# yhw-yhw/TalkSHOW

Hardware: NVIDIA H100
Metric: smplx_motion_frames_per_sec (higher is better)
Workload: dtype f32

## Files before the change

### talkshow_b200/csrc/api.cu

```cuda
#include "convstack.h"
#include "pixelcnn.h"

using namespace ts;

static std::string g_create_err;

float* ts_engine::upload(const std::vector<float>& h) {
  if (host_only) return nullptr;
  void* d = dmalloc(h.size() * sizeof(float));
  TS_CUDA(cudaMemcpy(d, h.data(), h.size() * sizeof(float), cudaMemcpyHostToDevice));
  return (float*)d;
}
unsigned short* ts_engine::upload(const std::vector<unsigned short>& h) {
  if (host_only) return nullptr;
  void* d = dmalloc(h.size() * sizeof(unsigned short));
  TS_CUDA(cudaMemcpy(d, h.data(), h.size() * sizeof(unsigned short), cudaMemcpyHostToDevice));
  return (unsigned short*)d;
}
void* ts_engine::dmalloc(size_t bytes) {
  if (host_only) return nullptr;
  void* d = nullptr;
  TS_CUDA(cudaMalloc(&d, bytes ? bytes : 16));
  (alloc_sink ? *alloc_sink : owned).push_back(d);
  return d;
// ... 60 lines not shown

extern "C" int ts_set_pixelcnn_ctas(ts_engine* e, int n) {
  if (!e || n < 0) return TS_ERR_INVALID;
  e->pixel_ctas = n;
  return TS_OK;
}

extern "C" int ts_set_vq_parallel(ts_engine* e, int max_batch) {
  if (!e || max_batch < 0) return TS_ERR_INVALID;
  e->vq_parallel_batch = max_batch;
  return TS_OK;
}

extern "C" int ts_set_pixelcnn_fusion(ts_engine* e, int on) {
  if (!e) return TS_ERR_INVALID;
  if (on < 0 || on > 2) return TS_ERR_INVALID;
  e->pixel_fusion = on;
  return TS_OK;
}

__constant__ float c_lower_pose[33] = {0.0f, 0.0f, 0.0f, 0.0f, 0.0f, 0.0f, 3.0747f, -0.0158f, -0.0152f,
    -1.1826512813568115f, 0.23866955935955048f, 0.15146760642528534f, -1.2604516744613647f, -0.3160211145877838f,
    -0.1603458970785141f, 1.1654603481292725f, 0.0f, 0.0f, 1.2521806955337524f, 0.041598282754421234f,
    -0.06312154978513718f, 0.0f, 0.0f, 0.0f, 0.0f, 0.0f, 0.0f, 0.0f, 0.0f, 0.0f, 0.0f, 0.0f, 0.0f};

__device__ __forceinline__ void rot6d_to_aa(const float* __restrict__ p, float& ax, float& ay, float& az) {
  const float a1x = p[0], a1y = p[1], a1z = p[2], a2x = p[3], a2y = p[4], a2z = p[5];
  float n1 = fmaxf(sqrtf(a1x * a1x + a1y * a1y + a1z * a1z), 1e-12f);
  const float b1x = a1x / n1, b1y = a1y / n1, b1z = a1z / n1;
  const float d = b1x * a2x + b1y * a2y + b1z * a2z;
  float b2x = a2x - d * b1x, b2y = a2y - d * b1y, b2z = a2z - d * b1z;
// ... 215 lines not shown
```

### talkshow_b200/csrc/pixelcnn.cu

```cuda
#include "pixelcnn.h"
#include "convstack.h"

#include <algorithm>
#include <memory>
#include <cmath>

namespace ts {


struct Job {
  int epi, layer, col, nrows, K, ncol;
  bool pairs;
  int rofs = 0;
};

constexpr double PIX_ROWCOST = 0.0;

static int rows_cap(int K) { return std::min(PIX_MAXROWS, (PIX_WBUF / (K + 1)) & ~3); }

static void push_vert0(std::vector<std::vector<Job>>& st, int D, bool split) {
  if (split) {
    st.push_back({{EPI_VERT0, 0, 0, 2 * D, 6 * D, 1, true}});
    st.push_back({{EPI_VERT0, 0, 1, 2 * D, 6 * D, 1, true}});
  } else {
// ... 13 lines not shown
  }
  for (int c = 0; c < 2; ++c) {
    std::vector<Job> j = {{EPI_HRESF, 0, c, D, D, 1, false}};
    if (c == 0) j.push_back({EPI_V2H, L - 1, 0, 2 * D, 2 * D, 2, false});
    st.push_back(j);
    st.push_back({{EPI_HGATE, 1, c, 2 * D, c ? 2 * D : D, 1, true}});
    for (int l = 2; l < L; ++l)
      st.push_back({{EPI_HGATE2, l, c, 2 * D, c ? 3 * D : 2 * D, 1, true}, {EPI_HRES, l - 1, c, D, D, 1, false}});
    st.push_back({{EPI_OUT1F, 0, c, 512, 2 * D, 1, false}});
    for (int q = 0; q < out2_split; ++q) st.push_back({{EPI_OUT2, 0, c, PIX_NCODE / out2_split, 512, 1, false, q * (PIX_NCODE / out2_split)}});
    st.push_back({{EPI_SAMPLE, 0, c, 0, c == 0 ? 1 : 0, 1, false}});
  }
  return st;
}

static std::vector<std::vector<Job>> build_stages_fused2(int L, int D = PIX_D, int out2_split = 1, bool v0_split = false) {
  std::vector<std::vector<Job>> st;
  push_vert0(st, D, v0_split);
  st.push_back({{EPI_FUSEV, 0, 0, D, D, 2, false}, {EPI_V2H, 0, 0, 2 * D, 2 * D, 2, false}});
  for (int l = 1; l < L; ++l) {
    std::vector<Job> j = {{EPI_VERT, l, 0, 2 * D, 4 * D, 1, true}, {EPI_VERT, l, 1, 2 * D, 4 * D, 1, true}};
    if (l == 1) j.push_back({EPI_HGATE, 0, 0, 2 * D, 0, 1, true});
    st.push_back(j);
  }
  for (int c = 0; c < 2; ++c) {
    st.push_back({{EPI_HRESF, 0, c, D, D, 1, false}, {EPI_V2H1, 1, c, 2 * D, 2 * D, 1, false}});
    {
      std::vector<Job> j = {{EPI_HGATE, 1, c, 2 * D, c ? 2 * D : D, 1, true}};
      if (L > 2) j.push_back({EPI_V2H1, 2, c, 2 * D, 2 * D, 1, false});
      st.push_back(j);
// ... 22 lines not shown
  for (int c = 0; c < 2; ++c) {
    std::vector<Job> j = {{EPI_HGATE, 0, c, 2 * D, c ? D : 0, 1, true}};
    if (c == 0) j.push_back({EPI_V2H, L - 1, 0, 2 * D, 2 * D, 2, false});
    st.push_back(j);
    st.push_back({{EPI_HRES, 0, c, D, D, 1, false}});
    st.push_back({{EPI_FUSEH, 0, c, D, D, 1, false}});
    for (int l = 1; l < L; ++l) {
      st.push_back({{EPI_HGATE, l, c, 2 * D, c ? 2 * D : D, 1, true}});
      st.push_back({{EPI_HRES, l, c, D, D, 1, false}});
    }
    st.push_back({{EPI_OUT1, 0, c, 512, D, 1, false}});
    st.push_back({{EPI_OUT2, 0, c, PIX_NCODE, 512, 1, false}});
    st.push_back({{EPI_SAMPLE, 0, c, 0, 0, 1, false}});
  }
  return st;
}

static PixLayout make_layout(int L, int hvslots, int MB = PIX_MB) {
  PixLayout a;
  int o = 0;
  auto take = [&](int nseg) { int r = o; o += nseg * PIX_D * MB; return r; };
  a.E = take(4 * 2);
  a.XV1P = take(2);
  a.XV = take(L * 2 * 2);
  a.HV = take(hvslots * 2 * 2);
  a.V2H = take(L * 2 * 2);
  a.G = take(2);
  a.XHP = take(1);
  a.XH = take(2 * (L + 1));
  a.Y = take(2);
// ... 150 lines not shown
  if (e->pixel_ctas > 0) {
    if (e->pixel_ctas < PIX_MB || e->pixel_ctas > e->sm_count) {
      const int n = e->pixel_ctas, sms = e->sm_count;
      fail(TS_ERR_UNSUPPORTED, "pixelcnn plan: ts_set_pixelcnn_ctas(%d) outside [%d, %d] (one CTA per sample of a 64-sample tile; SM count)", n, PIX_MB, sms);
    }
    P->ncta = e->pixel_ctas & ~1;
  }
  if (const char* v = getenv("TS_PIX_CTAS")) {
    const int n = atoi(v);
    if (n >= PIX_MB && n <= e->sm_count) P->ncta = n;
  }
  P->cl = cl;
  P->nclasses = ncls;
  bool fused = level >= 1 && L >= 3;
  P->sched = fused ? level : 0;
  P->lay = make_layout(L, P->sched == 2 ? L : 2);
  if (P->ncta < PIX_MB) fail(TS_ERR_UNSUPPORTED, "pixelcnn plan needs >= %d SMs (have %d)", PIX_MB, P->ncta);
  P->fused = fused;
  const int out2_split = (PIX_NCODE + PIX_MAXROWS * P->ncta - 1) / (PIX_MAXROWS * P->ncta);
  if (out2_split > 1 && !fused) fail(TS_ERR_UNSUPPORTED, "pixelcnn plan: %d CTAs need the fused plan", P->ncta);
  const bool v0_split = fused && 2 * cdiv(2 * D, rows_cap(6 * D)) > P->ncta / cl;
  auto stages = P->sched == 2 ? build_stages_fused2(L, PIX_D, out2_split, v0_split)
                : fused       ? build_stages_fused(L, PIX_D, out2_split, v0_split)
                              : build_stages(L);
  P->nstages = (int)stages.size();
  if (P->nstages > 160) fail(TS_ERR_UNSUPPORTED, "pixelcnn plan: %d stages per row (> 160)", P->nstages);
  P->table.assign((size_t)P->nstages * P->ncta, PixTask{0, 0, 0, 0, 0, 0, 0, 0});
  WeightSrc ws(ck, L);
  if (fused) ws.build_fused();
  int64_t dense = 0;
  int t0_ofs = 0;
  if (fused) {
    const float* ew = ck.f32("embedding.weight", {PIX_NCODE, D});
    const Job j0{EPI_HGATE, 0, 1, 2 * D, D, 1, true};
    P->blob.resize((size_t)PIX_NCODE * 2 * D);
    std::vector<float> wrow((size_t)2 * D * D), brow(2 * D);
    for (int jr = 0; jr < 2 * D; ++jr) {
      brow[jr] = ws.bias(j0, jr);
      for (int k = 0; k < D; ++k) wrow[(size_t)jr * D + k] = ws.w(j0, jr, k);
    }
    for (int code = 0; code < PIX_NCODE; ++code)
      for (int jr = 0; jr < 2 * D; ++jr) {
        double a = 0.0;
        for (int k = 0; k < D; ++k) a += (double)wrow[(size_t)jr * D + k] * (double)ew[(size_t)code * D + k];
        P->blob[(size_t)code * 2 * D + jr] = (float)(a + (double)brow[jr]);
      }
  }
  const size_t table_floats = P->blob.size();
  for (int s = 0; s < P->nstages; ++s) {
    auto& jobs = stages[s];
    if (jobs[0].epi == EPI_SAMPLE) {
      for (int c = 0; c < P->ncta; ++c)
        P->table[(size_t)s * P->ncta + c] = PixTask{EPI_SAMPLE, 0, jobs[0].col, 0, 0, jobs[0].K ? t0_ofs : 0, jobs[0].K, 0};
      continue;
    }
    std::vector<double> cost;
    double tot = 0;
    const double alpha = getenv("TS_PIX_ROWCOST") ? atof(getenv("TS_PIX_ROWCOST")) : PIX_ROWCOST;
    for (auto& j : jobs) { double c = (double)j.nrows * (j.K ? std::max(j.K, 256) + alpha : 16) * j.ncol; cost.push_back(c); tot += c; }
    std::vector<int> nc(jobs.size()), lo(jobs.size());
    int used = 0;
    const int nunit = P->ncta / cl;
    const int rowcap = PIX_MAXROWS;
    for (size_t i = 0; i < jobs.size(); ++i) {
      const int cap = jobs[i].K ? rows_cap(jobs[i].K / cl) : 4 * PIX_MAXROWS;
      lo[i] = (jobs[i].nrows + cap - 1) / cap;
      nc[i] = std::max(lo[i], (int)std::floor(nunit * cost[i] / tot));
      used += nc[i];
    }
    for (size_t i = 0; used < nunit; i = (i + 1) % jobs.size()) { nc[i]++; used++; }
    while (used > nunit) {
      size_t big = 0; int slack = -1;
      for (size_t i = 0; i < jobs.size(); ++i) if (nc[i] - lo[i] > slack) { slack = nc[i] - lo[i]; big = i; }
      if (slack <= 0) fail(TS_ERR_UNSUPPORTED, "pixelcnn plan: %d SMs are too few for stage %d", P->ncta, s);
      nc[big]--; used--;
    }
    int cta = 0;
    for (size_t i = 0; i < jobs.size(); ++i) {
      const Job& j = jobs[i];
      const int unit = j.pairs ? 2 : 1, units = j.nrows / unit;
      const int base = units / nc[i], rem = units % nc[i];
      int u0 = 0;
      for (int q = 0; q < nc[i]; ++q) {
        int nu = base + (q < rem ? 1 : 0);
        for (int rank = 0; rank < cl; ++rank, ++cta) {
          PixTask t{0, 0, 0, 0, 0, 0, 0, 0};
          if (nu > 0) {
            t.epi = j.epi; t.layer = j.layer; t.col = j.col;
            t.row0 = j.rofs + u0 * unit; t.nrows = nu * unit; t.K = j.K; t.rpad = (t.nrows + 3) & ~3;
            if (t.K > 0 && t.nrows > rowcap) fail(TS_ERR_UNSUPPORTED, "pixelcnn plan: %d rows per unit (> %d) with %d SMs", t.nrows, rowcap, P->ncta);
            const int Ks = t.K / cl, k0 = rank * Ks;
            size_t sz = (size_t)(Ks + 1) * t.rpad;
            if (sz > (size_t)PIX_WBUF) fail(TS_ERR_UNSUPPORTED, "pixelcnn plan: task blob %zu floats > staging buffer", sz);
            t.wofs = (int)P->blob.size();
            P->blob.resize(P->blob.size() + sz, 0.f);
            float* dst = P->blob.data() + t.wofs;
            for (int r = 0; r < t.nrows; ++r) {
              for (int k = 0; k < Ks; ++k) dst[(size_t)k * t.rpad + r] = ws.w(j, t.row0 - j.rofs + r, k0 + k);
              dst[(size_t)Ks * t.rpad + r] = ws.bias(j, t.row0 - j.rofs + r);
            }
            dense += (int64_t)t.nrows * Ks;
          }
          P->table[(size_t)s * P->ncta + cta] = t;
        }
        u0 += nu;
      }
    }
  }
  P->staged_row_bytes = 4 * ((int64_t)(P->blob.size() - table_floats) + 3LL * D * D);
  (void)dense;
  P->has_v1 = true;

  if (!e->host_only) {
    P->d_table = (PixTask*)e->dmalloc(P->table.size() * sizeof(PixTask));
    TS_CUDA(cudaMemcpy(P->d_table, P->table.data(), P->table.size() * sizeof(PixTask), cudaMemcpyHostToDevice));
    P->d_blob = e->upload(P->blob);
    const float* ew = ck.f32("embedding.weight", {PIX_NCODE, D});
    P->d_emb = e->upload(std::vector<float>(ew, ew + (size_t)PIX_NCODE * D));
    std::vector<float> cls((size_t)L * ncls * 2 * D);
// ... 19 lines not shown
  const int64_t* pre;
  int64_t* idx_out;
  float* logits_out;
  unsigned* barrier;
  PixLayout lay;
  int B, T0, Ttot, log_r0, L, nstages, ncta, fused;
  unsigned long long* trace;
  int trace_row;
  float temperature;
  int top_k;
  float* logp_out;
  float top_p, min_p;
  int* kept_out;
  const int64_t* seeds;
  const int64_t* anchors;
};

__device__ __forceinline__ uint32_t smem_u32(const void* p) { return (uint32_t)__cvta_generic_to_shared(p); }
__device__ __forceinline__ void mbar_init(uint64_t* bar, int count) {
  asm volatile("mbarrier.init.shared::cta.b64 [%0], %1;" ::"r"(smem_u32(bar)), "r"(count));
}
__device__ __forceinline__ void mbar_expect_tx(uint64_t* bar, uint32_t bytes) {
  asm volatile("mbarrier.arrive.expect_tx.shared::cta.b64 _, [%0], %1;" ::"r"(smem_u32(bar)), "r"(bytes) : "memory");
}
__device__ __forceinline__ void mbar_wait(uint64_t* bar, uint32_t parity) {
  asm volatile(
      "{\n"
      ".reg .pred p;\n"
      "WAIT_LOOP:\n"
      "mbarrier.try_wait.parity.shared::cta.b64 p, [%0], %1;\n"
// ... 322 lines not shown
__device__ __forceinline__ float sigmoidf_(float x) { return 1.0f / (1.0f + expf(-x)); }

struct EpiPre {
  float a, b;
  bool valid;
};

template <int MB, bool S2 = false>
__device__ __forceinline__ EpiPre prefetch_epilogue(const PixTask& t, const PixArgs& A, int r) {
  constexpr int SEG = PIX_D * MB;
  EpiPre p;
  p.a = 0.f; p.b = 0.f; p.valid = false;
  if constexpr (S2) {
    if (t.epi == EPI_HGATE || t.epi == EPI_HGATE2) return p;
  }
  const int tid = threadIdx.x, m = tid & (MB - 1), j = tid / MB;
  const PixLayout& a = A.lay;
  if (t.epi == EPI_HGATE || t.epi == EPI_HGATE2) {
    if (j < (t.nrows >> 1) && (t.nrows >> 1) * MB <= PIX_THREADS) {
      const int q = (t.row0 >> 1) + j;
      const float* v2h = A.arena + a.V2H + ((t.layer * 2 + t.col) * 2) * SEG;
      p.a = __ldcg(v2h + ax<MB>(q, m));
      p.b = __ldcg(v2h + ax<MB>(PIX_D + q, m));
      p.valid = true;
    }
  } else if (t.epi == EPI_HRES && t.layer > 0 && !A.fused) {
    if (j < t.nrows && t.nrows * MB <= PIX_THREADS) {
      p.a = __ldcg(A.arena + a.XH + (t.col * (A.L + 1) + t.layer) * SEG + ax<MB>(t.row0 + j, m));
      p.valid = true;
    }
// ... 528 lines not shown
  } else {
    code = A.pre[((size_t)m * A.T0 + r) * 2 + c];
  }
  if (r >= A.T0 && tid == 0) A.idx_out[((size_t)m * (A.Ttot - A.T0) + (r - A.T0)) * 2 + c] = code;
  A.arena[A.lay.E + ((r & 3) * 2 + c) * SEG + ax<MB>(tid, m)] = A.emb[(size_t)code * PIX_D + tid];
  if (t.K) {
    const float2 tw = *reinterpret_cast<const float2*>(A.blob + t.wofs + (size_t)code * (2 * PIX_D) + 2 * tid);
    const float* v2h = A.arena + A.lay.V2H + ((0 * 2 + 1) * 2) * SEG;
    const float* cls = A.arena + A.lay.CLS;
    const float zt = (__ldcg(v2h + ax<MB>(tid, m)) + tw.x) + cls[ax<MB>(tid, m)];
    const float zs = (__ldcg(v2h + ax<MB>(PIX_D + tid, m)) + tw.y) + cls[ax<MB>(PIX_D + tid, m)];
    A.arena[A.lay.G + ax<MB>(tid, m)] = tanhf(zt) * sigmoidf_(zs);
  }
}

constexpr int PIX_MAXSTAGES = 160;
constexpr size_t PIX_SMEM = (size_t)(2 * PIX_WBUF + 8 * PIX_MAXROWS * 64) * sizeof(float) + 64 + PIX_MAXSTAGES * sizeof(PixTask);

__device__ __forceinline__ unsigned long long globaltimer_ns() {
  unsigned long long t;
  asm volatile("mov.u64 %0, %%globaltimer;" : "=l"(t));
  return t;
}

template <bool PERSISTENT, int PIPE, bool TRACE = false, bool S2 = false, int MB = 64, bool WARP = false>
__global__ void __launch_bounds__(PIX_THREADS, 1) pixelcnn_kernel(PixArgs A, int r_single, int s_single) {
  extern __shared__ __align__(128) unsigned char smem_raw[];
  float* wbuf = reinterpret_cast<float*>(smem_raw);
  float* red = wbuf + 2 * PIX_WBUF;
  uint64_t* bars = reinterpret_cast<uint64_t*>(red + 8 * PIX_MAXROWS * 64);
  PixTask* tasks = reinterpret_cast<PixTask*>(bars + 8);
// ... 7 lines not shown
    for (int i = tid; i < nf; i += PIX_THREADS) wbuf[i] = A.blob[t.wofs + i];
    __syncthreads();
    EpiPre pre; pre.a = pre.b = 0.f; pre.valid = false;
    run_matmul_task<0, MB, S2>(t, A, r_single, wbuf, red, pre);
    return;
  }

  if (tid == 0) {
    mbar_init(&bars[0], 1);
    mbar_init(&bars[1], 1);
    asm volatile("fence.mbarrier_init.release.cluster;" ::: "memory");
  }
  for (int i = tid; i < A.nstages * 8; i += PIX_THREADS)
    reinterpret_cast<int*>(tasks)[i] = reinterpret_cast<const int*>(A.table + (size_t)(i >> 3) * A.ncta + cta)[i & 7];
  __syncthreads();
  uint32_t uses[2] = {0u, 0u};
  const int total = A.Ttot * A.nstages;
  if (tid == 0) {
    const PixTask t0 = tasks[0];
    if (task_active(t0, 0, A.log_r0) && t0.epi != EPI_SAMPLE) {
      mbar_expect_tx(&bars[0], task_bytes(t0));
      tma_load_1d(wbuf, A.blob + t0.wofs, task_bytes(t0), &bars[0]);
    }
  }
  int r = 0, s = 0;
  for (int g = 0; g < total; ++g) {
    const PixTask t = tasks[s];
    const int buf = g & 1;
    if (tid == 0 && g + 1 < total) {
      int s1 = s + 1, r1 = r;
      if (s1 == A.nstages) { s1 = 0; r1 = r + 1; }
      const PixTask tn = tasks[s1];
      if (task_active(tn, r1, A.log_r0) && tn.epi != EPI_SAMPLE) {
        fence_proxy_async();
        mbar_expect_tx(&bars[buf ^ 1], task_bytes(tn));
        tma_load_1d(wbuf + (buf ^ 1) * PIX_WBUF, A.blob + tn.wofs, task_bytes(tn), &bars[buf ^ 1]);
      }
    }
    const bool active = task_active(t, r, A.log_r0);
    const bool has_w = active && t.epi != EPI_SAMPLE;
    EpiPre pre;
    pre.a = pre.b = 0.f; pre.valid = false;
    if (active && t.epi != EPI_SAMPLE) pre = prefetch_epilogue<MB, S2>(t, A, r);
    float qpre[8];
    if (active && t.epi == EPI_SAMPLE && cta < A.B && r >= A.T0 && (!WARP || A.temperature > 0.f))
      draw_noise(A, r, t.col, cta, qpre);
    if (has_w) { mbar_wait(&bars[buf], uses[buf] & 1u); uses[buf]++; }
    unsigned long long* tr = nullptr;
    if constexpr (TRACE) {
      if (tid == 0 && r == A.trace_row && A.trace) { tr = A.trace + ((size_t)s * A.ncta + cta) * 4; tr[0] = globaltimer_ns(); }
    }
    if (g > 0) grid_wait(A.barrier, (unsigned)g * (unsigned)A.ncta);
    if constexpr (TRACE) { if (tr) tr[1] = globaltimer_ns(); }
    if (active) {
      if (t.epi == EPI_SAMPLE) {
        if (cta < A.B) run_sample_task<MB, true, WARP>(t, A, r, cta, red, qpre);
      }
      else run_matmul_task<PIPE, MB, S2>(t, A, r, wbuf + buf * PIX_WBUF, red, pre);
    }
    if constexpr (TRACE) { __syncthreads(); if (tr) tr[2] = globaltimer_ns(); }
    grid_arrive(A.barrier);
    if constexpr (TRACE) { if (tr) tr[3] = globaltimer_ns(); }
    if (++s == A.nstages) { s = 0; ++r; }
  }
}

#include "pixelcnn3.inc"

__global__ void build_cls_kernel(const float* __restrict__ cls_w, const int64_t* __restrict__ label, float* arena, int cls_off,
                                 int L, int ncls, int B, int MB) {
  int n = L * 2 * PIX_D * MB;
  for (int i = blockIdx.x * blockDim.x + threadIdx.x; i < n; i += gridDim.x * blockDim.x) {
    int m = i % MB, ch = (i / MB) % (2 * PIX_D), l = i / (2 * PIX_D * MB);
    float v = 0.f;
    if (m < B) {
      long long lb = label[m];
// ... 16 lines not shown
  if (e->ws.sizing) return;
  split_codes_kernel<<<cdiv(B * T, 256), 256, 0, s>>>(idx, idx_c, codes_out, B * T);
  e->launches++;
  TS_CUDA(cudaGetLastError());
}

__global__ void logits_to_ref_kernel(const float* __restrict__ in, float* __restrict__ out, int B, int T) {
  long n = (long)2 * T * B * PIX_NCODE;
  for (long i = blockIdx.x * (long)blockDim.x + threadIdx.x; i < n; i += (long)gridDim.x * blockDim.x) {
    int code = i % PIX_NCODE;
    long sb = i / PIX_NCODE;
    int b = sb % B, step = sb / B;
    int t = step >> 1, c = step & 1;
    out[(((long)b * PIX_NCODE + code) * T + t) * 2 + c] = in[i];
  }
}

static void generate_chunk(ts_engine* e, const Act3& aud, int b0, const int64_t* label, const float* noise, int noise_B,
                           int64_t* idx_out, float* logits_out, int B, int T, const int64_t* pre, int T0, cudaStream_t s,
                           bool logits_all, const SampleCtl* ctl, const int64_t* seeds, const int64_t* anchors) {
  PixelPlan* P = e->pix;
  Plan3* Q = (Plan3*)P->p3;
  const int Ttot = T0 + T, D = P->D;
  const bool v3 = (e->pixel_mode == 2 && Q) || !P->has_v1;
  float* a_emb = e->ws.alloc<float>((size_t)B * Ttot * D);
  float* audv = e->ws.alloc<float>((size_t)B * Ttot * D);
  float* audh = e->ws.alloc<float>((size_t)B * Ttot * D);
  const int MB3 = v3 ? c3_pick_mb(Q, B) : 0;
  float* arena3 = v3 ? e->ws.alloc<float>((size_t)((B + MB3 - 1) / MB3) * make_layout3(Q->L, Q->D, MB3).total) : nullptr;
  if (e->ws.sizing) return;
// ... 12 lines not shown
  (void)noise_B;

  if (v3) {
    launch_pixelcnn3(e, P, Q, audv, audh, label, noise, idx_out, logits_out, B, T0, Ttot, pre, logits_all, arena3, MB3, s, ctl, seeds,
                     anchors);
    return;
  }
  if (B > PIX_MB)
    fail(TS_ERR_UNSUPPORTED, "pixelcnn: the grid-wide executor takes %d samples per call (got %d); the host shim chunks larger batches", PIX_MB, B);
  int MB = B <= 16 ? 16 : B <= 32 ? 32 : 64;
  if (const char* v = getenv("TS_PIX_TILE")) {
    const int t = atoi(v);
    if ((t == 8 || t == 16 || t == 32 || t == 64) && t >= B) MB = t;
  }
  const bool tracing = P->d_trace && P->trace_row >= 0;
  if (P->sched == 2 || (tracing && MB != 16)) MB = 64;
  const PixLayout lay = make_layout(P->L, P->sched == 2 ? P->L : 2, MB);
  TS_CUDA(cudaMemsetAsync(P->d_arena, 0, (size_t)lay.total * sizeof(float), s));
  TS_CUDA(cudaMemsetAsync(P->d_barrier, 0, 4096, s));
  build_cls_kernel<<<e->sm_count, 256, 0, s>>>(P->d_cls, label, P->d_arena, lay.CLS, P->L, P->nclasses, B, MB);
  e->launches++;
  TS_CUDA(cudaGetLastError());

  PixArgs A;
  A.table = P->d_table; A.blob = P->d_blob; A.arena = P->d_arena; A.emb = P->d_emb;
  A.audv = audv; A.audh = audh; A.noise = noise; A.pre = pre; A.idx_out = idx_out; A.logits_out = logits_out;
  A.barrier = P->d_barrier; A.lay = lay;
  A.B = B; A.T0 = T0; A.Ttot = Ttot; A.log_r0 = logits_all ? 0 : T0; A.L = P->L; A.nstages = P->nstages; A.ncta = P->ncta;
  A.fused = P->fused ? 1 : 0;
  A.trace = P->d_trace; A.trace_row = P->trace_row;
  const SampleCtl c = ctl ? *ctl : SampleCtl();
  A.temperature = c.temperature; A.top_k = c.top_k; A.logp_out = c.logp_out;
  A.top_p = c.top_p; A.min_p = c.min_p; A.kept_out = c.kept_out;
  A.seeds = seeds;
  A.anchors = anchors;
  if (e->pixel_mode == 0) {
    static const int pipe = getenv("TS_PIX_PIPE") ? atoi(getenv("TS_PIX_PIPE")) : 5;
    void* fn = pipe == 0 ? (void*)pixelcnn_kernel<true, 0> : pipe == 4 ? (void*)pixelcnn_kernel<true, 4> : (void*)pixelcnn_kernel<true, 5>;
    if (MB == 32) fn = (void*)pixelcnn_kernel<true, 5, false, false, 32>;
    if (MB == 16) fn = (void*)pixelcnn_kernel<true, 5, false, false, 16>;
    if (MB == 8) fn = (void*)pixelcnn_kernel<true, 5, false, false, 8>;
    if (tracing) fn = MB == 16 ? (void*)pixelcnn_kernel<true, 5, true, false, 16> : (void*)pixelcnn_kernel<true, 5, true>;
    if (P->sched == 2) fn = tracing ? (void*)pixelcnn_kernel<true, 5, true, true> : (void*)pixelcnn_kernel<true, 5, false, true>;
    if (ctl) {
      fn = MB == 8 ? (void*)pixelcnn_kernel<true, 5, false, false, 8, true>
           : MB == 16 ? (void*)pixelcnn_kernel<true, 5, false, false, 16, true>
           : MB == 32 ? (void*)pixelcnn_kernel<true, 5, false, false, 32, true>
           : P->sched == 2 ? (void*)pixelcnn_kernel<true, 5, false, true, 64, true>
                           : (void*)pixelcnn_kernel<true, 5, false, false, 64, true>;
    }
    TS_CUDA(cudaFuncSetAttribute(fn, cudaFuncAttributeMaxDynamicSharedMemorySize, (int)PIX_SMEM));
    int rs = 0, ss = 0;
    void* args[] = {&A, &rs, &ss};
    if (P->timing) TS_CUDA(cudaEventRecord(P->ev0, s));
    if (P->ncta < e->sm_count && (P->ncta & 1) == 0) {
      cudaLaunchConfig_t cfg = {};
      cfg.gridDim = dim3(P->ncta);
      cfg.blockDim = dim3(PIX_THREADS);
      cfg.dynamicSmemBytes = PIX_SMEM;
      cfg.stream = s;
      cudaLaunchAttribute at[2];
      at[0].id = cudaLaunchAttributeClusterDimension;
      at[0].val.clusterDim.x = 2; at[0].val.clusterDim.y = 1; at[0].val.clusterDim.z = 1;
      at[1].id = cudaLaunchAttributeCooperative;
      at[1].val.cooperative = 1;
// ... 5 lines not shown
    }
    if (P->timing) { TS_CUDA(cudaEventRecord(P->ev1, s)); P->timed_rows += Ttot; P->timed_launches++; P->pending = true; }
    e->launches++;
  } else {
    void (*fn1)(PixArgs, int, int) = P->sched == 2 ? pixelcnn_kernel<false, 0, false, true> : pixelcnn_kernel<false, 0>;
    if (MB == 32) fn1 = pixelcnn_kernel<false, 0, false, false, 32>;
    if (MB == 16) fn1 = pixelcnn_kernel<false, 0, false, false, 16>;
    if (MB == 8) fn1 = pixelcnn_kernel<false, 0, false, false, 8>;
    if (ctl) {
      fn1 = MB == 8 ? pixelcnn_kernel<false, 0, false, false, 8, true>
            : MB == 16 ? pixelcnn_kernel<false, 0, false, false, 16, true>
            : MB == 32 ? pixelcnn_kernel<false, 0, false, false, 32, true>
            : P->sched == 2 ? pixelcnn_kernel<false, 0, false, true, 64, true>
                            : pixelcnn_kernel<false, 0, false, false, 64, true>;
    }
    TS_CUDA(cudaFuncSetAttribute(fn1, cudaFuncAttributeMaxDynamicSharedMemorySize, (int)PIX_SMEM));
    for (int r = 0; r < Ttot; ++r)
      for (int st = 0; st < P->nstages; ++st) {
        fn1<<<P->ncta, PIX_THREADS, PIX_SMEM, s>>>(A, r, st);
        e->launches++;
      }
    TS_CUDA(cudaGetLastError());
  }
}

void pixel_destroy(ts_engine* e) {
  if (!e->pix) return;
  delete (Plan3*)e->pix->p3;
  tf_free(e->pix->tf);
  delete e->pix;
// ... 122 lines not shown
  *nstages = e->pix->nstages;
  *ncta = e->pix->ncta;
  TS_API_END(e)
}

extern "C" int ts_debug_pixelcnn_plan(ts_engine* e, int32_t* table, int64_t* table_len, float* blob, int64_t* blob_len) {
  TS_API_BEGIN(e)
  if (!e->pix) fail(TS_ERR_NOT_LOADED, "pixelcnn weights not loaded");
  PixelPlan* P = e->pix;
  const int64_t hdr = 32;
  const int64_t tl = hdr + (int64_t)P->table.size() * 8, bl = (int64_t)P->blob.size();
  if (table) {
    if (*table_len < tl) fail(TS_ERR_INVALID, "table buffer too small");
    int32_t h[32] = {P->ncta, P->nstages, P->L, PIX_D, PIX_MB, P->lay.E, P->lay.XV1P, P->lay.XV, P->lay.HV, P->lay.V2H,
                     P->lay.G, P->lay.XHP, P->lay.XH, P->lay.Y, P->lay.LOG, P->lay.CLS, P->lay.total, PIX_NCODE, P->cl,
                     P->sched == 2 ? P->L : 2};
    memcpy(table, h, sizeof h);
    memcpy(table + hdr, P->table.data(), P->table.size() * sizeof(PixTask));
  }
  if (blob) {
    if (*blob_len < bl) fail(TS_ERR_INVALID, "blob buffer too small");
    memcpy(blob, P->blob.data(), P->blob.size() * sizeof(float));
  }
  *table_len = tl;
  *blob_len = bl;
  TS_API_END(e)
}

static void check_pix(ts_engine* e, int B, int T) {
  if (!e->pix) fail(TS_ERR_NOT_LOADED, "pixelcnn weights not loaded");
  if (e->host_only) fail(TS_ERR_UNSUPPORTED, "host-only engine cannot execute");
// ... 119 lines not shown
```

### talkshow_b200/csrc/pixelcnn.h

```cpp
#pragma once
#include "kernels.h"

namespace ts {

constexpr int PIX_D = 256;
constexpr int PIX_MB = 64;
constexpr int PIX_SEG = PIX_D * PIX_MB;
constexpr int PIX_THREADS = 256;
constexpr int PIX_MAXROWS = 16;
constexpr int PIX_WBUF = 18560;
constexpr int PIX_NCODE = 2048;

enum PixEpi {
  EPI_IDLE = 0,
  EPI_VERT0 = 1,
  EPI_VERT = 2,
  EPI_V2H = 3,
  EPI_FUSEV = 4,
  EPI_HGATE = 5,
  EPI_HRES = 6,
  EPI_FUSEH = 7,
  EPI_OUT1 = 8,
  EPI_OUT2 = 9,
  EPI_SAMPLE = 10,
  EPI_HRESF = 11,
  EPI_HGATE2 = 12,
// ... 5 lines not shown
  int epi, layer, col, row0, nrows, wofs, K, rpad;
};

struct PixLayout {
  int E, XV1P, XV, HV, V2H, G, XHP, XH, Y, LOG, CLS, total;
};

struct PixelPlan {
  int L = 0, ncta = 0, nstages = 0, nclasses = 4;
  int D = PIX_D;
  bool has_v1 = false;
  int cl = 1;
  bool fused = false;
  int sched = 1;
  PixLayout lay;
  std::vector<PixTask> table;
  std::vector<float> blob;
  int64_t row_bytes = 0;
  int64_t staged_row_bytes = 0;
  PixTask* d_table = nullptr;
  float* d_blob = nullptr;
  float* d_emb = nullptr;
  float* d_cls = nullptr;
  float* d_arena = nullptr;
  unsigned* d_barrier = nullptr;
  Layer emb_aud, fuse_v_a, fuse_h_a;
  void* p3 = nullptr;
  void* tf = nullptr;
  unsigned long long* d_trace = nullptr;
  int trace_row = -1;
// ... 34 lines not shown
```

### talkshow_b200/pipeline.py

```python
from __future__ import annotations

import torch

from .engine import Engine, check_anchors, resolve_clip_seeds, sample_controls
from .nets.base import draw_sampler_noise


def shard_range(B, rank, world):
    base, rem = divmod(B, world)
    lo = rank * base + min(rank, rem)
    return lo, lo + base + (1 if rank < rem else 0)


class WholeBody:

    def __init__(self, engine: Engine, overlap_batch=64, overlap_ctas=96):
        self.e = engine
        self.device = engine.device
        self.overlap_batch = overlap_batch if not getattr(engine, "host_only", True) else 0
        self.overlap_ctas = overlap_ctas
        self.e2 = None
        self._side = None
        self._body_engine = engine

    def load(self, pixel_ckpt, vq_ckpt, face_ckpt):
        self.e.load_pixelcnn(pixel_ckpt["generator"])
        self.e.load_audioenc(pixel_ckpt["audioencoder"])
        self.e.load_vq(0, vq_ckpt["g_body"])
        self.e.load_vq(1, vq_ckpt["g_hand"])
        self.e.load_face(face_ckpt["generator"])
        dim = pixel_ckpt["generator"]["embedding.weight"].shape[1]
        if self.overlap_batch > 0 and dim == 256 and self.overlap_ctas < self.e.sm_count:
            idx = self.device.index or 0
            self.e2 = Engine(idx)
            self.e2.set_pixelcnn_ctas(self.overlap_ctas)
            self.e2.load_pixelcnn(pixel_ckpt["generator"])
            self.e2.load_audioenc(pixel_ckpt["audioencoder"])
            self.e2.load_vq(0, vq_ckpt["g_body"])
            self.e2.load_vq(1, vq_ckpt["g_hand"])
            self._side = torch.cuda.Stream(device=self.device, priority=-1)

    @property
    def launches(self):
        return self.e.launches + (self.e2.launches if self.e2 is not None else 0)

    def pixelcnn_timing(self, enable=True):
        self.e.pixelcnn_timing(enable)
        if self.e2 is not None:
            self.e2.pixelcnn_timing(enable)

# ... 151 lines not shown
```

Before: 249,500.

## Add skewed PixelCNN schedule overlapping horizontal chain with vertical layers

Adds a new schedule level (3) that skews the horizontal-stack chain for column 0 so it runs alongside the vertical-stack layers, which cuts the number of grid-wide barriers per latent row. Stages that need more CTAs than are available are bin-packed into several sub-rows that run back to back inside a CTA under a local __syncthreads instead of a grid barrier. The TMA weight prefetch is reworked to track its own load counter across these rows. Level 3 becomes the pipeline default, which brings extra planning complexity, more table rows, and some risk of load imbalance.

```diff
diff --git a/talkshow_b200/csrc/api.cu b/talkshow_b200/csrc/api.cu
--- a/talkshow_b200/csrc/api.cu
+++ b/talkshow_b200/csrc/api.cu
@@ -98,7 +98,7 @@
 
 extern "C" int ts_set_pixelcnn_fusion(ts_engine* e, int on) {
   if (!e) return TS_ERR_INVALID;
-  if (on < 0 || on > 2) return TS_ERR_INVALID;
+  if (on < 0 || on > 3) return TS_ERR_INVALID;
   e->pixel_fusion = on;
   return TS_OK;
 }
diff --git a/talkshow_b200/csrc/pixelcnn.cu b/talkshow_b200/csrc/pixelcnn.cu
--- a/talkshow_b200/csrc/pixelcnn.cu
+++ b/talkshow_b200/csrc/pixelcnn.cu
@@ -51,6 +51,46 @@
   return st;
 }
 
+static std::vector<std::vector<Job>> build_stages_skewed(int L, int D = PIX_D, int out2_split = 1, bool v0_split = false) {
+  std::vector<std::vector<Job>> chain;
+  chain.push_back({{EPI_HGATE, 0, 0, 2 * D, 0, 1, true}});
+  chain.push_back({{EPI_HRESF, 0, 0, D, D, 1, false}});
+  chain.push_back({{EPI_HGATE, 1, 0, 2 * D, D, 1, true}});
+  for (int l = 2; l < L; ++l) chain.push_back({{EPI_HGATE2, l, 0, 2 * D, 2 * D, 1, true}, {EPI_HRES, l - 1, 0, D, D, 1, false}});
+  auto v2h1 = [&](int l, int c) { return Job{EPI_V2H1, l, c, 2 * D, 2 * D, 1, false}; };
+  std::vector<std::vector<Job>> st;
+  push_vert0(st, D, v0_split);
+  st.push_back({{EPI_FUSEV, 0, 0, D, D, 2, false}, {EPI_V2H, 0, 0, 2 * D, 2 * D, 2, false}});
+  for (int l = 1; l < L; ++l) {
+    std::vector<Job> j = {{EPI_VERT, l, 0, 2 * D, 4 * D, 1, true}, {EPI_VERT, l, 1, 2 * D, 4 * D, 1, true}};
+    if (l >= 2) j.push_back(v2h1(l - 1, 0));
+    j.insert(j.end(), chain[l - 1].begin(), chain[l - 1].end());
+    st.push_back(j);
+  }
+  for (int k = L - 1; k <= L; ++k) {
+    std::vector<Job> j = chain[k];
+    if (k == L - 1) j.insert(j.begin(), v2h1(L - 1, 0));
+    st.push_back(j);
+  }
+  for (int c = 0; c < 2; ++c) {
+    if (c == 1) {
+      st.push_back({{EPI_HRESF, 0, 1, D, D, 1, false}, v2h1(1, 1)});
+      std::vector<Job> j = {{EPI_HGATE, 1, 1, 2 * D, 2 * D, 1, true}};
+      if (L > 2) j.push_back(v2h1(2, 1));
+      st.push_back(j);
+      for (int l = 2; l < L; ++l) {
+        std::vector<Job> g = {{EPI_HGATE2, l, 1, 2 * D, 3 * D, 1, true}, {EPI_HRES, l - 1, 1, D, D, 1, false}};
+        if (l + 1 < L) g.push_back(v2h1(l + 1, 1));
+        st.push_back(g);
+      }
+    }
+    st.push_back({{EPI_OUT1F, 0, c, 512, 2 * D, 1, false}});
+    for (int q = 0; q < out2_split; ++q) st.push_back({{EPI_OUT2, 0, c, PIX_NCODE / out2_split, 512, 1, false, q * (PIX_NCODE / out2_split)}});
+    st.push_back({{EPI_SAMPLE, 0, c, 0, c == 0 ? 1 : 0, 1, false}});
+  }
+  return st;
+}
+
 static std::vector<std::vector<Job>> build_stages_fused2(int L, int D = PIX_D, int out2_split = 1, bool v0_split = false) {
   std::vector<std::vector<Job>> st;
   push_vert0(st, D, v0_split);
@@ -103,6 +143,69 @@
     st.push_back({{EPI_SAMPLE, 0, c, 0, 0, 1, false}});
   }
   return st;
+}
+
+static double job_cost(const Job& j, int rows, double alpha) { return (double)rows * (j.K ? std::max(j.K, 256) + alpha : 16) * j.ncol; }
+
+constexpr double PIX_TASKCOST = 16.0 * 256.0;
+
+struct SubTask { int job, u0, nu; };
+
+static std::vector<std::vector<SubTask>> pack_stage(const std::vector<Job>& jobs, const std::vector<int>& lo, int nunit, double alpha) {
+  const size_t nj = jobs.size();
+  auto units = [&](size_t i) { return jobs[i].nrows / (jobs[i].pairs ? 2 : 1); };
+  auto cost = [&](const Job& j, int nu) { return job_cost(j, nu * (j.pairs ? 2 : 1), alpha) + PIX_TASKCOST; };
+  auto pack = [&](const std::vector<int>& nt, std::vector<std::vector<SubTask>>* out) -> double {
+    std::vector<std::pair<double, SubTask>> tasks;
+    for (size_t i = 0; i < nj; ++i) {
+      const int n = units(i), base = n / nt[i], rem = n % nt[i];
+      for (int q = 0, u0 = 0; q < nt[i]; ++q) {
+        const int nu = base + (q < rem ? 1 : 0);
+        tasks.push_back({cost(jobs[i], nu), SubTask{(int)i, u0, nu}});
+        u0 += nu;
+      }
+    }
+    std::stable_sort(tasks.begin(), tasks.end(), [](const auto& a, const auto& b) { return a.first > b.first; });
+    std::vector<double> load(nunit, 0.0);
+    std::vector<std::vector<SubTask>> cta(nunit);
+    for (auto& [c, t] : tasks) {
+      int best = -1;
+      for (int u = 0; u < nunit; ++u)
+        if ((int)cta[u].size() < PIX_MAXSUB && (best < 0 || load[u] < load[best])) best = u;
+      if (best < 0) return INFINITY;
+      load[best] += c;
+      cta[best].push_back(t);
+    }
+    if (out) *out = std::move(cta);
+    return *std::max_element(load.begin(), load.end());
+  };
+  std::vector<size_t> order(nj);
+  for (size_t i = 0; i < nj; ++i) order[i] = i;
+  std::stable_sort(order.begin(), order.end(), [&](size_t a, size_t b) {
+    return job_cost(jobs[a], jobs[a].nrows, alpha) < job_cost(jobs[b], jobs[b].nrows, alpha);
+  });
+  std::vector<int> nt = lo;
+  double span = pack(nt, nullptr);
+  for (int pass = 0; pass < 4; ++pass) {
+    bool moved = false;
+    for (size_t i : order) {
+      const int n0 = nt[i], nu = units(i);
+      int pick = n0;
+      for (int n = lo[i]; n <= nu; ++n) {
+        if (n > lo[i] && (nu + n - 1) / n == (nu + n - 2) / (n - 1)) continue;
+        if (n == n0) continue;
+        nt[i] = n;
+        const double sp = pack(nt, nullptr);
+        if (sp < span) { span = sp; pick = n; }
+      }
+      nt[i] = pick;
+      moved = moved || pick != n0;
+    }
+    if (!moved) break;
+  }
+  std::vector<std::vector<SubTask>> out;
+  if (!std::isfinite(pack(nt, &out))) out.clear();
+  return out;
 }
 
 static PixLayout make_layout(int L, int hvslots, int MB = PIX_MB) {
@@ -283,18 +386,24 @@
   P->nclasses = ncls;
   bool fused = level >= 1 && L >= 3;
   P->sched = fused ? level : 0;
-  P->lay = make_layout(L, P->sched == 2 ? L : 2);
+  P->lay = make_layout(L, P->sched >= 2 ? L : 2);
   if (P->ncta < PIX_MB) fail(TS_ERR_UNSUPPORTED, "pixelcnn plan needs >= %d SMs (have %d)", PIX_MB, P->ncta);
   P->fused = fused;
   const int out2_split = (PIX_NCODE + PIX_MAXROWS * P->ncta - 1) / (PIX_MAXROWS * P->ncta);
   if (out2_split > 1 && !fused) fail(TS_ERR_UNSUPPORTED, "pixelcnn plan: %d CTAs need the fused plan", P->ncta);
   const bool v0_split = fused && 2 * cdiv(2 * D, rows_cap(6 * D)) > P->ncta / cl;
-  auto stages = P->sched == 2 ? build_stages_fused2(L, PIX_D, out2_split, v0_split)
+  auto stages = P->sched == 3 ? build_stages_skewed(L, PIX_D, out2_split, v0_split)
+                : P->sched == 2 ? build_stages_fused2(L, PIX_D, out2_split, v0_split)
                 : fused       ? build_stages_fused(L, PIX_D, out2_split, v0_split)
                               : build_stages(L);
-  P->nstages = (int)stages.size();
-  if (P->nstages > 160) fail(TS_ERR_UNSUPPORTED, "pixelcnn plan: %d stages per row (> 160)", P->nstages);
-  P->table.assign((size_t)P->nstages * P->ncta, PixTask{0, 0, 0, 0, 0, 0, 0, 0});
+  P->nbar = (int)stages.size();
+  P->nstages = 0;
+  P->table.clear();
+  auto new_row = [&]() {
+    if (P->nstages == PIX_MAXSTAGES) fail(TS_ERR_UNSUPPORTED, "pixelcnn plan: more than %d table rows per latent row", PIX_MAXSTAGES);
+    P->table.resize(P->table.size() + P->ncta, PixTask{0, 0, 0, 0, 0, 0, 0, 0});
+    return P->nstages++;
+  };
   WeightSrc ws(ck, L);
   if (fused) ws.build_fused();
   int64_t dense = 0;
@@ -316,26 +425,66 @@
       }
   }
   const size_t table_floats = P->blob.size();
-  for (int s = 0; s < P->nstages; ++s) {
+  const int rowcap = PIX_MAXROWS;
+  auto make_task = [&](const Job& j, int u0, int nu, int rank) {
+    const int unit = j.pairs ? 2 : 1;
+    PixTask t{0, 0, 0, 0, 0, 0, 0, 0};
+    if (nu > 0) {
+      t.epi = j.epi; t.layer = j.layer; t.col = j.col;
+      t.row0 = j.rofs + u0 * unit; t.nrows = nu * unit; t.K = j.K; t.rpad = (t.nrows + 3) & ~3;
+      if (t.K > 0 && t.nrows > rowcap) fail(TS_ERR_UNSUPPORTED, "pixelcnn plan: %d rows per unit (> %d) with %d SMs", t.nrows, rowcap, P->ncta);
+      const int Ks = t.K / cl, k0 = rank * Ks;
+      size_t sz = (size_t)(Ks + 1) * t.rpad;
+      if (sz > (size_t)PIX_WBUF) fail(TS_ERR_UNSUPPORTED, "pixelcnn plan: task blob %zu floats > staging buffer", sz);
+      t.wofs = (int)P->blob.size();
+      P->blob.resize(P->blob.size() + sz, 0.f);
+      float* dst = P->blob.data() + t.wofs;
+      for (int r = 0; r < t.nrows; ++r) {
+        for (int k = 0; k < Ks; ++k) dst[(size_t)k * t.rpad + r] = ws.w(j, t.row0 - j.rofs + r, k0 + k);
+        dst[(size_t)Ks * t.rpad + r] = ws.bias(j, t.row0 - j.rofs + r);
+      }
+      dense += (int64_t)t.nrows * Ks;
+    }
+    return t;
+  };
+  for (int s = 0; s < P->nbar; ++s) {
     auto& jobs = stages[s];
     if (jobs[0].epi == EPI_SAMPLE) {
+      const int row = new_row();
       for (int c = 0; c < P->ncta; ++c)
-        P->table[(size_t)s * P->ncta + c] = PixTask{EPI_SAMPLE, 0, jobs[0].col, 0, 0, jobs[0].K ? t0_ofs : 0, jobs[0].K, 0};
+        P->table[(size_t)row * P->ncta + c] = PixTask{EPI_SAMPLE, 0, jobs[0].col, 0, 0, jobs[0].K ? t0_ofs : 0, jobs[0].K, 0};
       continue;
     }
     std::vector<double> cost;
     double tot = 0;
     const double alpha = getenv("TS_PIX_ROWCOST") ? atof(getenv("TS_PIX_ROWCOST")) : PIX_ROWCOST;
-    for (auto& j : jobs) { double c = (double)j.nrows * (j.K ? std::max(j.K, 256) + alpha : 16) * j.ncol; cost.push_back(c); tot += c; }
+    for (auto& j : jobs) { double c = job_cost(j, j.nrows, alpha); cost.push_back(c); tot += c; }
     std::vector<int> nc(jobs.size()), lo(jobs.size());
-    int used = 0;
+    int used = 0, need = 0;
     const int nunit = P->ncta / cl;
-    const int rowcap = PIX_MAXROWS;
     for (size_t i = 0; i < jobs.size(); ++i) {
       const int cap = jobs[i].K ? rows_cap(jobs[i].K / cl) : 4 * PIX_MAXROWS;
       lo[i] = (jobs[i].nrows + cap - 1) / cap;
       nc[i] = std::max(lo[i], (int)std::floor(nunit * cost[i] / tot));
       used += nc[i];
+      need += lo[i];
+    }
+    if (P->sched == 3 && need > nunit) {
+      const auto per = pack_stage(jobs, lo, nunit, alpha);
+      if (per.empty()) fail(TS_ERR_UNSUPPORTED, "pixelcnn plan: %d SMs are too few for stage %d", P->ncta, s);
+      size_t nsub = 0;
+      for (auto& v : per) nsub = std::max(nsub, v.size());
+      for (size_t k = 0; k < nsub; ++k) {
+        const int row = new_row();
+        if (k + 1 < nsub) P->cont[row >> 5] |= 1u << (row & 31);
+        for (int u = 0; u < nunit; ++u) {
+          if (k >= per[u].size()) continue;
+          const SubTask& st = per[u][k];
+          for (int rank = 0; rank < cl; ++rank)
+            P->table[(size_t)row * P->ncta + u * cl + rank] = make_task(jobs[st.job], st.u0, st.nu, rank);
+        }
+      }
+      continue;
     }
     for (size_t i = 0; used < nunit; i = (i + 1) % jobs.size()) { nc[i]++; used++; }
     while (used > nunit) {
@@ -344,6 +493,7 @@
       if (slack <= 0) fail(TS_ERR_UNSUPPORTED, "pixelcnn plan: %d SMs are too few for stage %d", P->ncta, s);
       nc[big]--; used--;
     }
+    const int row = new_row();
     int cta = 0;
     for (size_t i = 0; i < jobs.size(); ++i) {
       const Job& j = jobs[i];
@@ -352,26 +502,8 @@
       int u0 = 0;
       for (int q = 0; q < nc[i]; ++q) {
         int nu = base + (q < rem ? 1 : 0);
-        for (int rank = 0; rank < cl; ++rank, ++cta) {
-          PixTask t{0, 0, 0, 0, 0, 0, 0, 0};
-          if (nu > 0) {
-            t.epi = j.epi; t.layer = j.layer; t.col = j.col;
-            t.row0 = j.rofs + u0 * unit; t.nrows = nu * unit; t.K = j.K; t.rpad = (t.nrows + 3) & ~3;
-            if (t.K > 0 && t.nrows > rowcap) fail(TS_ERR_UNSUPPORTED, "pixelcnn plan: %d rows per unit (> %d) with %d SMs", t.nrows, rowcap, P->ncta);
-            const int Ks = t.K / cl, k0 = rank * Ks;
-            size_t sz = (size_t)(Ks + 1) * t.rpad;
-            if (sz > (size_t)PIX_WBUF) fail(TS_ERR_UNSUPPORTED, "pixelcnn plan: task blob %zu floats > staging buffer", sz);
-            t.wofs = (int)P->blob.size();
-            P->blob.resize(P->blob.size() + sz, 0.f);
-            float* dst = P->blob.data() + t.wofs;
-            for (int r = 0; r < t.nrows; ++r) {
-              for (int k = 0; k < Ks; ++k) dst[(size_t)k * t.rpad + r] = ws.w(j, t.row0 - j.rofs + r, k0 + k);
-              dst[(size_t)Ks * t.rpad + r] = ws.bias(j, t.row0 - j.rofs + r);
-            }
-            dense += (int64_t)t.nrows * Ks;
-          }
-          P->table[(size_t)s * P->ncta + cta] = t;
-        }
+        for (int rank = 0; rank < cl; ++rank, ++cta)
+          P->table[(size_t)row * P->ncta + cta] = make_task(j, u0, nu, rank);
         u0 += nu;
       }
     }
@@ -421,6 +553,7 @@
   int* kept_out;
   const int64_t* seeds;
   const int64_t* anchors;
+  unsigned cont[PIX_MAXSTAGES / 32];
 };
 
 __device__ __forceinline__ uint32_t smem_u32(const void* p) { return (uint32_t)__cvta_generic_to_shared(p); }
@@ -773,6 +906,7 @@
   if constexpr (S2) {
     if (t.epi == EPI_HGATE || t.epi == EPI_HGATE2) return p;
   }
+  if (t.epi == EPI_HGATE && t.col == 0 && t.layer == 0) return p;
   const int tid = threadIdx.x, m = tid & (MB - 1), j = tid / MB;
   const PixLayout& a = A.lay;
   if (t.epi == EPI_HGATE || t.epi == EPI_HGATE2) {
@@ -1331,7 +1465,6 @@
   }
 }
 
-constexpr int PIX_MAXSTAGES = 160;
 constexpr size_t PIX_SMEM = (size_t)(2 * PIX_WBUF + 8 * PIX_MAXROWS * 64) * sizeof(float) + 64 + PIX_MAXSTAGES * sizeof(PixTask);
 
 __device__ __forceinline__ unsigned long long globaltimer_ns() {
@@ -1369,43 +1502,43 @@
   for (int i = tid; i < A.nstages * 8; i += PIX_THREADS)
     reinterpret_cast<int*>(tasks)[i] = reinterpret_cast<const int*>(A.table + (size_t)(i >> 3) * A.ncta + cta)[i & 7];
   __syncthreads();
-  uint32_t uses[2] = {0u, 0u};
+  int nw = 0;
+  int ni = 0, gi = 0;
+  unsigned nbar = 0;
+  bool bar_pending = false;
   const int total = A.Ttot * A.nstages;
-  if (tid == 0) {
-    const PixTask t0 = tasks[0];
-    if (task_active(t0, 0, A.log_r0) && t0.epi != EPI_SAMPLE) {
-      mbar_expect_tx(&bars[0], task_bytes(t0));
-      tma_load_1d(wbuf, A.blob + t0.wofs, task_bytes(t0), &bars[0]);
-    }
-  }
   int r = 0, s = 0;
   for (int g = 0; g < total; ++g) {
     const PixTask t = tasks[s];
-    const int buf = g & 1;
-    if (tid == 0 && g + 1 < total) {
-      int s1 = s + 1, r1 = r;
-      if (s1 == A.nstages) { s1 = 0; r1 = r + 1; }
-      const PixTask tn = tasks[s1];
-      if (task_active(tn, r1, A.log_r0) && tn.epi != EPI_SAMPLE) {
-        fence_proxy_async();
-        mbar_expect_tx(&bars[buf ^ 1], task_bytes(tn));
-        tma_load_1d(wbuf + (buf ^ 1) * PIX_WBUF, A.blob + tn.wofs, task_bytes(tn), &bars[buf ^ 1]);
-      }
-    }
     const bool active = task_active(t, r, A.log_r0);
     const bool has_w = active && t.epi != EPI_SAMPLE;
+    if (tid == 0) {
+      const int want = nw + 1 + (has_w ? 1 : 0);
+      while (ni < want && gi < total) {
+        const int ri = gi / A.nstages, si = gi - ri * A.nstages;
+        const PixTask tn = tasks[si];
+        if (task_active(tn, ri, A.log_r0) && tn.epi != EPI_SAMPLE) {
+          fence_proxy_async();
+          mbar_expect_tx(&bars[ni & 1], task_bytes(tn));
+          tma_load_1d(wbuf + (ni & 1) * PIX_WBUF, A.blob + tn.wofs, task_bytes(tn), &bars[ni & 1]);
+          ++ni;
+        }
+        ++gi;
+      }
+    }
     EpiPre pre;
     pre.a = pre.b = 0.f; pre.valid = false;
     if (active && t.epi != EPI_SAMPLE) pre = prefetch_epilogue<MB, S2>(t, A, r);
     float qpre[8];
     if (active && t.epi == EPI_SAMPLE && cta < A.B && r >= A.T0 && (!WARP || A.temperature > 0.f))
       draw_noise(A, r, t.col, cta, qpre);
-    if (has_w) { mbar_wait(&bars[buf], uses[buf] & 1u); uses[buf]++; }
+    const int buf = nw & 1;
+    if (has_w) { mbar_wait(&bars[buf], (nw >> 1) & 1); }
     unsigned long long* tr = nullptr;
     if constexpr (TRACE) {
       if (tid == 0 && r == A.trace_row && A.trace) { tr = A.trace + ((size_t)s * A.ncta + cta) * 4; tr[0] = globaltimer_ns(); }
     }
-    if (g > 0) grid_wait(A.barrier, (unsigned)g * (unsigned)A.ncta);
+    if (bar_pending) grid_wait(A.barrier, nbar * (unsigned)A.ncta);
     if constexpr (TRACE) { if (tr) tr[1] = globaltimer_ns(); }
     if (active) {
       if (t.epi == EPI_SAMPLE) {
@@ -1413,8 +1546,16 @@
       }
       else run_matmul_task<PIPE, MB, S2>(t, A, r, wbuf + buf * PIX_WBUF, red, pre);
     }
+    if (has_w) ++nw;
     if constexpr (TRACE) { __syncthreads(); if (tr) tr[2] = globaltimer_ns(); }
-    grid_arrive(A.barrier);
+    const bool cont = (A.cont[s >> 5] >> (s & 31)) & 1u;
+    if (cont) {
+      __syncthreads();
+    } else {
+      grid_arrive(A.barrier);
+      ++nbar;
+    }
+    bar_pending = !cont;
     if constexpr (TRACE) { if (tr) tr[3] = globaltimer_ns(); }
     if (++s == A.nstages) { s = 0; ++r; }
   }
@@ -1461,6 +1602,20 @@
     int t = step >> 1, c = step & 1;
     out[(((long)b * PIX_NCODE + code) * T + t) * 2 + c] = in[i];
   }
+}
+
+template <bool PERSISTENT>
+static void (*skew_kernel(int MB, bool warp))(PixArgs, int, int) {
+  constexpr int PIPE = PERSISTENT ? 5 : 0;
+  if (warp)
+    return MB == 8 ? pixelcnn_kernel<PERSISTENT, PIPE, false, true, 8, true>
+           : MB == 16 ? pixelcnn_kernel<PERSISTENT, PIPE, false, true, 16, true>
+           : MB == 32 ? pixelcnn_kernel<PERSISTENT, PIPE, false, true, 32, true>
+                      : pixelcnn_kernel<PERSISTENT, PIPE, false, true, 64, true>;
+  return MB == 8 ? pixelcnn_kernel<PERSISTENT, PIPE, false, true, 8>
+         : MB == 16 ? pixelcnn_kernel<PERSISTENT, PIPE, false, true, 16>
+         : MB == 32 ? pixelcnn_kernel<PERSISTENT, PIPE, false, true, 32>
+                    : pixelcnn_kernel<PERSISTENT, PIPE, false, true, 64>;
 }
 
 static void generate_chunk(ts_engine* e, const Act3& aud, int b0, const int64_t* label, const float* noise, int noise_B,
@@ -1503,8 +1658,8 @@
     if ((t == 8 || t == 16 || t == 32 || t == 64) && t >= B) MB = t;
   }
   const bool tracing = P->d_trace && P->trace_row >= 0;
-  if (P->sched == 2 || (tracing && MB != 16)) MB = 64;
-  const PixLayout lay = make_layout(P->L, P->sched == 2 ? P->L : 2, MB);
+  if (P->sched == 2 || (tracing && (MB != 16 || P->sched == 3))) MB = 64;
+  const PixLayout lay = make_layout(P->L, P->sched >= 2 ? P->L : 2, MB);
   TS_CUDA(cudaMemsetAsync(P->d_arena, 0, (size_t)lay.total * sizeof(float), s));
   TS_CUDA(cudaMemsetAsync(P->d_barrier, 0, 4096, s));
   build_cls_kernel<<<e->sm_count, 256, 0, s>>>(P->d_cls, label, P->d_arena, lay.CLS, P->L, P->nclasses, B, MB);
@@ -1523,6 +1678,7 @@
   A.top_p = c.top_p; A.min_p = c.min_p; A.kept_out = c.kept_out;
   A.seeds = seeds;
   A.anchors = anchors;
+  std::copy(P->cont, P->cont + PIX_MAXSTAGES / 32, A.cont);
   if (e->pixel_mode == 0) {
     static const int pipe = getenv("TS_PIX_PIPE") ? atoi(getenv("TS_PIX_PIPE")) : 5;
     void* fn = pipe == 0 ? (void*)pixelcnn_kernel<true, 0> : pipe == 4 ? (void*)pixelcnn_kernel<true, 4> : (void*)pixelcnn_kernel<true, 5>;
@@ -1538,6 +1694,7 @@
            : P->sched == 2 ? (void*)pixelcnn_kernel<true, 5, false, true, 64, true>
                            : (void*)pixelcnn_kernel<true, 5, false, false, 64, true>;
     }
+    if (P->sched == 3) fn = (tracing && !ctl) ? (void*)pixelcnn_kernel<true, 5, true, true> : (void*)skew_kernel<true>(MB, ctl != nullptr);
     TS_CUDA(cudaFuncSetAttribute(fn, cudaFuncAttributeMaxDynamicSharedMemorySize, (int)PIX_SMEM));
     int rs = 0, ss = 0;
     void* args[] = {&A, &rs, &ss};
@@ -1573,6 +1730,7 @@
             : P->sched == 2 ? pixelcnn_kernel<false, 0, false, true, 64, true>
                             : pixelcnn_kernel<false, 0, false, false, 64, true>;
     }
+    if (P->sched == 3) fn1 = skew_kernel<false>(MB, ctl != nullptr);
     TS_CUDA(cudaFuncSetAttribute(fn1, cudaFuncAttributeMaxDynamicSharedMemorySize, (int)PIX_SMEM));
     for (int r = 0; r < Ttot; ++r)
       for (int st = 0; st < P->nstages; ++st) {
@@ -1725,7 +1883,11 @@
     if (*table_len < tl) fail(TS_ERR_INVALID, "table buffer too small");
     int32_t h[32] = {P->ncta, P->nstages, P->L, PIX_D, PIX_MB, P->lay.E, P->lay.XV1P, P->lay.XV, P->lay.HV, P->lay.V2H,
                      P->lay.G, P->lay.XHP, P->lay.XH, P->lay.Y, P->lay.LOG, P->lay.CLS, P->lay.total, PIX_NCODE, P->cl,
-                     P->sched == 2 ? P->L : 2};
+                     P->sched >= 2 ? P->L : 2};
+    if (P->nbar != P->nstages) {
+      h[20] = P->nbar;
+      memcpy(h + 21, P->cont, sizeof P->cont);
+    }
     memcpy(table, h, sizeof h);
     memcpy(table + hdr, P->table.data(), P->table.size() * sizeof(PixTask));
   }
diff --git a/talkshow_b200/csrc/pixelcnn.h b/talkshow_b200/csrc/pixelcnn.h
--- a/talkshow_b200/csrc/pixelcnn.h
+++ b/talkshow_b200/csrc/pixelcnn.h
@@ -10,6 +10,8 @@
 constexpr int PIX_MAXROWS = 16;
 constexpr int PIX_WBUF = 18560;
 constexpr int PIX_NCODE = 2048;
+constexpr int PIX_MAXSTAGES = 160;
+constexpr int PIX_MAXSUB = 3;
 
 enum PixEpi {
   EPI_IDLE = 0,
@@ -45,6 +47,8 @@
   bool fused = false;
   int sched = 1;
   PixLayout lay;
+  int nbar = 0;
+  unsigned cont[PIX_MAXSTAGES / 32] = {};
   std::vector<PixTask> table;
   std::vector<float> blob;
   int64_t row_bytes = 0;
diff --git a/talkshow_b200/pipeline.py b/talkshow_b200/pipeline.py
--- a/talkshow_b200/pipeline.py
+++ b/talkshow_b200/pipeline.py
@@ -14,8 +14,9 @@
 
 class WholeBody:
 
-    def __init__(self, engine: Engine, overlap_batch=64, overlap_ctas=96):
+    def __init__(self, engine: Engine, overlap_batch=64, overlap_ctas=96, pixel_fusion=3):
         self.e = engine
+        self.pixel_fusion = pixel_fusion
         self.device = engine.device
         self.overlap_batch = overlap_batch if not getattr(engine, "host_only", True) else 0
         self.overlap_ctas = overlap_ctas
@@ -24,6 +25,8 @@
         self._body_engine = engine
 
     def load(self, pixel_ckpt, vq_ckpt, face_ckpt):
+        if hasattr(self.e, "set_pixelcnn_fusion"):
+            self.e.set_pixelcnn_fusion(self.pixel_fusion)
         self.e.load_pixelcnn(pixel_ckpt["generator"])
         self.e.load_audioenc(pixel_ckpt["audioencoder"])
         self.e.load_vq(0, vq_ckpt["g_body"])
@@ -34,6 +37,7 @@
             idx = self.device.index or 0
             self.e2 = Engine(idx)
             self.e2.set_pixelcnn_ctas(self.overlap_ctas)
+            self.e2.set_pixelcnn_fusion(self.pixel_fusion)
             self.e2.load_pixelcnn(pixel_ckpt["generator"])
             self.e2.load_audioenc(pixel_ckpt["audioencoder"])
             self.e2.load_vq(0, vq_ckpt["g_body"])
```

After: 254,300, median of 6. 1.02x the previous value.
